# timsu1104/Open-vocabulary-3D-Object-Detection

Measured on AMD Instinct MI355X. Metric: scenes/sec (train step) SUN RGB-D 20k pts nqueries=128, higher is better.
Workload: dtype bf16; 1 GPU; SUN RGB-D train step, bs=8/GPU, 20000 pts, nqueries=128, 3DETR 256-d enc3/dec8, text-emb 640, AdamW + clip 0.1; global_batch=8, points=20000, parallelism=dp1

## Files before the change

include/ov3d.h:

```cpp
#ifndef OV3D_H_
#define OV3D_H_

#include <stdint.h>

#ifdef __cplusplus
extern "C" {
#endif

#define OV3D_OK 0
#define OV3D_EINVAL (-1)
#define OV3D_ELAUNCH (-2)

const char* ov3d_version(void);

int ov3d_fps(const float* xyz, int B, int N, int M, int32_t* idx_out, float* new_xyz_out,
             float* workspace, void* stream);
long long ov3d_fps_workspace(int B, int N);
int ov3d_fps_pair_status(const float* workspace, int B, int N, int M, int32_t* status,
                         void* stream);

int ov3d_nbr_max_fwd(const void* y, long long P, int S, int C, void* out, uint8_t* arg,
                     void* stream);
int ov3d_nbr_max_bwd(const void* g, const uint8_t* arg, long long P, int S, int C, void* dy,
                     void* stream);
// ... 195 lines not shown
int ov3d_rows256_supported(long long M, int N, int K);
int ov3d_rows256(const void* X, long long ldx, int K, int N, const void* W, long long ldw, void* Y,
                 long long ldy, long long M, unsigned int* counters, void* stream);
int ov3d_rows256_bn(const void* X, long long ldx, const float* scale, const float* shift,
                    const void* W, long long ldw, void* Y, long long ldy, void* Z, long long ldz,
                    long long M, unsigned int* counters, void* stream);

typedef struct {
    const void* W;
    long long ldw;
    const void* bias;
    void* out;
    long long ldo;
    int N;
    int sel;
} ov3d_lngemm_problem;
int ov3d_lngemm_supported(int R, int C, int N);
int ov3d_lngemm_fwd(int R, const void* src, int src_bf16, const void* y, float dropout_p,
                    const int64_t* seed, int site, const float* ga, const float* ba,
                    const void* pos, int pos_bf16, const float* gb, const float* bb, float eps,
                    float* s, float* mean, float* rstd, void* xa, void* xap, void* xb, int xb_bf16,
                    long long xb_inner, long long xb_s0, long long xb_s1, int nprob,
                    const ov3d_lngemm_problem* probs, int epilogue, float dropout_p2,
                    const int64_t* seed2, int site2, void* stream);
int ov3d_lngemm_bwd_parts(int R);
int ov3d_lngemm_stamps_arm(void* buf);
int ov3d_lngemm_bwd(int R, const float* s, const float* mean, const float* rstd, const float* ds,
                    const void* dxa, const void* dxap, const void* dxb, int dxb_bf16,
                    long long dxb_inner, long long dxb_s0, long long dxb_s1, const float* ga,
                    const float* gb, float dropout_p, const int64_t* seed, int site, float* dsrc,
                    void* dy, void* dpos, int dpos_bf16, float* partials, int accumulate,
                    const void* W, long long ldw, int N, int epilogue, float dropout_p2,
                    const void* H, long long ldh, void* dx, long long lddx, void* stream);

int ov3d_attn_fwd(const void* q, const void* k, const void* v, long long sq, long long sk,
                  long long sv, int B, int H, int Lq, int Lk, float scale, float dropout_p,
                  const int64_t* seed, int site, void* o, long long so, float* lse,
                  uint32_t* dropbits, float* workspace, int nsplit, void* stream);
long long ov3d_attn_fwd_workspace(int B, int H, int Lq, int Lk, int nsplit);
long long ov3d_attn_dropbits_words(int B, int H, int Lq, int Lk);
int ov3d_attn_bwd(const void* q, const void* k, const void* v, long long sq, long long sk,
                  long long sv, const void* o, long long so, const void* dout, long long sdo,
                  const float* lse, int B, int H, int Lq, int Lk, float scale, float dropout_p,
                  const uint32_t* dropbits, float* dvec, void* dq, long long sdq, void* dk,
                  long long sdk, void* dv, long long sdv, float* workspace, int nsplit,
                  void* stream);

typedef struct {
    const void* q; long long sq; const void* k; long long sk; const void* v; long long sv;
    const void* dout; long long sdo; const float* lse; const float* dvec;
    const uint32_t* dropbits; void* dk; long long sdk; void* dv; long long sdv;
} ov3d_attn_dkdv_job;
int ov3d_attn_bwd_dkdv_batch(const ov3d_attn_dkdv_job* jobs, int njobs, int B, int H, int Lq,
                             int Lk, float scale, float dropout_p, void* stream);

int ov3d_attn_small_bwd(int on);

long long ov3d_attn_maskbits_words(int B, int Lq, int Lk);
int ov3d_attn_mask_pack(const void* src, int kind, float thr, int B, int Lq, int Lk,
                        uint32_t* words, void* stream);
int ov3d_attn_fwd_masked(const void* q, const void* k, const void* v, long long sq, long long sk,
                         long long sv, int B, int H, int Lq, int Lk, float scale, float dropout_p,
                         const int64_t* seed, int site, void* o, long long so, float* lse,
                         uint32_t* dropbits, float* workspace, int nsplit,
                         const uint32_t* maskbits, void* stream);
int ov3d_attn_fwd_pregen(const void* q, const void* k, const void* v, long long sq, long long sk,
// ... 267 lines not shown
```

open-vocabulary-3d-object-detection_amd/_native.py:

```python
import ctypes
import os

import torch

_HERE = os.path.dirname(os.path.abspath(__file__))
LIB_PATH = os.path.join(_HERE, "lib", "libov3d_hip.so")

OV3D_GIOU_CYTHON = 0
OV3D_GIOU_TENSOR = 1

_lib = None

_SIGS = {
    "ov3d_fps": "piiipppp",
    "ov3d_fps_pair_status": "piiipp",
    "ov3d_ball_query": "ppiiifipp",
    "ov3d_ball_query_cells": "ppiiifipplp",
    "ov3d_group_fwd": "ppplllpiiiiifipp",
    "ov3d_group_bwd": "ppiiiiilllpp",
    "ov3d_gather_fwd": "ppiiiipp",
    "ov3d_gather_bwd": "ppiiiipp",
    "ov3d_giou3d": "pppiiiiipipp",
    "ov3d_giou3d_bwd_aligned": "pppiiippp",
    "ov3d_giou3d_bwd": "pppiiiipppp",
# ... 65 lines not shown
    "ov3d_resnorm_bwd": "lipppppppilllppfpippipipippppip",
    "ov3d_rows_gemm": "iiiplplipplp",
    "ov3d_bn_stats_finalize": "piidppffpppppppp",
    "ov3d_colsum_group": "pipiip",
    "ov3d_sa_dy_fused": "ppppiiiipppppppppppip",
    "ov3d_sa_dy2_fused": "pppppppppppppppiiipppip",
    "ov3d_bn_bwd_stats_finalize": "piidppppppppp",
    "ov3d_rows_gemm_act": "iiiplplipifpiplplp",
    "ov3d_rows_gemm_group": "iipip",
    "ov3d_tile_gemm": "iiiplplipplp",
    "ov3d_tile_gemm_act": "iiiplplipifpiplplp",
    "ov3d_tile_gemm2": "iiiplpliplpliplp",
    "ov3d_tile_gemm_batched": "iiiipllpllipllp",
    "ov3d_sun_aug_points": "pilippiipippp",
    "ov3d_sun_aug_boxes": "plpppiipipippp",
    "ov3d_sun_cuboid_eval": "piipppiiippippppp",
    "ov3d_sun_crop_sample": "piipppiippipppp",
    "ov3d_sun_labels": "pip",
    "ov3d_box_points_count": "pllipiipp",
    "ov3d_box3d_iou_eval": "ppppiiipp",
    "ov3d_ap_match": "ppppiiiidpp",
    "ov3d_ap_curve": "plppiplppp",
    "ov3d_project_box2d": "pppliipppppp",
    "ov3d_heads_out_fwd": "plippipiippippppppipp",
    "ov3d_heads_out_bwd": "pppiiiipiippppppplp",
    "ov3d_gemm256": "plplpiplpliiiip",
    "ov3d_conv3x3_gemm256": "piiiiplpiplpliip",
    "ov3d_gemm256_pair": "pplpplppippliiip",
    "ov3d_gemm256_batched": "pllpllpliplliiiiip",
    "ov3d_lngemm_fwd": "ipipfpipppippfppppppilllipifpip",
    "ov3d_rows256": "pliiplpllpp",
    "ov3d_rows256_bn": "plppplplpllpp",
    "ov3d_lngemm_bwd": "ipppppppilllppfpipppipipliifplplp",
}
EXPORTS = tuple(_SIGS) + ("ov3d_version", "ov3d_sa_layer_supported", "ov3d_attn_fwd_workspace",
                          "ov3d_attn_dropbits_words", "ov3d_attn_maskbits_words", "ov3d_fps_workspace", "ov3d_attn_small_bwd", "ov3d_set_loss_fwd_parts",
                          "ov3d_wgrad_workspace", "ov3d_wgrad_tiles", "ov3d_wgrad_group_tiles",
                          "ov3d_set_loss_desc_size",
                          "ov3d_resnorm_supported", "ov3d_resnorm_bwd_parts",
                          "ov3d_adamw_chunk", "ov3d_wgrad_group_workspace",
                          "ov3d_rows_gemm_supported", "ov3d_sa_dy_fused_supported",
                          "ov3d_tile_gemm_supported", "ov3d_sun_range_parts", "ov3d_heads_out_max_text",
                          "ov3d_heads_out_workspace", "ov3d_stamps_arm", "ov3d_stamps_count",
                          "ov3d_stamps_get", "ov3d_wall_clock_khz",
                          "ov3d_attnpool_fused_supported", "ov3d_lngemm_supported",
                          "ov3d_lngemm_bwd_parts", "ov3d_lngemm_stamps_arm", "ov3d_stream_create",
                          "ov3d_ball_query_ws_bytes", "ov3d_rows256_supported")

_CT = {"p": ctypes.c_void_p, "i": ctypes.c_int, "l": ctypes.c_longlong, "f": ctypes.c_float,
       "d": ctypes.c_double}


class NativeError(RuntimeError):
    pass


def load():
    global _lib
    if _lib is None:
        if not os.path.exists(LIB_PATH):
            raise NativeError(
                f"{LIB_PATH} not found: the HIP extension is required (no CPU fallback); "
                "build it with `make -C open-vocabulary-3d-object-detection_amd/csrc`")
        lib = ctypes.CDLL(LIB_PATH)
        for name, sig in _SIGS.items():
            fn = getattr(lib, name)
            fn.argtypes = [_CT[c] for c in sig]
            fn.restype = ctypes.c_int
        lib.ov3d_sa_layer_supported.argtypes = [ctypes.c_int, ctypes.c_int]
        lib.ov3d_sa_layer_supported.restype = ctypes.c_int
        lib.ov3d_attn_fwd_workspace.argtypes = [ctypes.c_int] * 5
        lib.ov3d_attn_fwd_workspace.restype = ctypes.c_longlong
        lib.ov3d_attn_dropbits_words.argtypes = [ctypes.c_int] * 4
        lib.ov3d_attn_dropbits_words.restype = ctypes.c_longlong
        lib.ov3d_set_loss_fwd_parts.argtypes = [ctypes.c_int] * 3
        lib.ov3d_set_loss_fwd_parts.restype = ctypes.c_longlong
        lib.ov3d_fps_workspace.argtypes = [ctypes.c_int] * 2
        lib.ov3d_fps_workspace.restype = ctypes.c_longlong
        lib.ov3d_stamps_arm.argtypes = [ctypes.c_void_p, ctypes.c_longlong, ctypes.c_longlong]
        lib.ov3d_stamps_arm.restype = ctypes.c_int
# ... 13 lines not shown
        lib.ov3d_wgrad_tiles.restype = ctypes.c_int
        lib.ov3d_wgrad_group_tiles.argtypes = [ctypes.c_int] * 2
        lib.ov3d_wgrad_group_tiles.restype = ctypes.c_int
        lib.ov3d_set_loss_desc_size.argtypes = []
        lib.ov3d_set_loss_desc_size.restype = ctypes.c_longlong
        lib.ov3d_resnorm_supported.argtypes = [ctypes.c_int]
        lib.ov3d_resnorm_supported.restype = ctypes.c_int
        lib.ov3d_resnorm_bwd_parts.argtypes = [ctypes.c_longlong, ctypes.c_int]
        lib.ov3d_resnorm_bwd_parts.restype = ctypes.c_int
        lib.ov3d_adamw_chunk.argtypes = []
        lib.ov3d_adamw_chunk.restype = ctypes.c_int
        lib.ov3d_wgrad_group_workspace.argtypes = [ctypes.c_void_p, ctypes.c_int]
        lib.ov3d_wgrad_group_workspace.restype = ctypes.c_longlong
        lib.ov3d_sa_dy_fused_supported.argtypes = [ctypes.c_int] * 2
        lib.ov3d_sa_dy_fused_supported.restype = ctypes.c_int
        lib.ov3d_rows_gemm_supported.argtypes = [ctypes.c_int] * 3
        lib.ov3d_rows256_supported.argtypes = [ctypes.c_longlong, ctypes.c_int, ctypes.c_int]
        lib.ov3d_rows256_supported.restype = ctypes.c_int
        lib.ov3d_rows_gemm_supported.restype = ctypes.c_int
        lib.ov3d_tile_gemm_supported.argtypes = [ctypes.c_int] * 3
        lib.ov3d_tile_gemm_supported.restype = ctypes.c_int
        lib.ov3d_sun_range_parts.argtypes = [ctypes.c_int]
        lib.ov3d_sun_range_parts.restype = ctypes.c_int
        lib.ov3d_heads_out_max_text.argtypes = []
        lib.ov3d_heads_out_max_text.restype = ctypes.c_int
        lib.ov3d_attnpool_fused_supported.argtypes = [ctypes.c_int] * 3
        lib.ov3d_attnpool_fused_supported.restype = ctypes.c_int
        lib.ov3d_lngemm_supported.argtypes = [ctypes.c_int] * 3
        lib.ov3d_lngemm_supported.restype = ctypes.c_int
        lib.ov3d_lngemm_bwd_parts.argtypes = [ctypes.c_int]
        lib.ov3d_lngemm_bwd_parts.restype = ctypes.c_int
        lib.ov3d_lngemm_stamps_arm.argtypes = [ctypes.c_void_p]
        lib.ov3d_lngemm_stamps_arm.restype = ctypes.c_int
        lib.ov3d_heads_out_workspace.argtypes = [ctypes.c_int] * 2
        lib.ov3d_heads_out_workspace.restype = ctypes.c_longlong
        lib.ov3d_stream_create.argtypes = [ctypes.c_void_p]
        lib.ov3d_ball_query_ws_bytes.argtypes = [ctypes.c_int] * 2
        lib.ov3d_ball_query_ws_bytes.restype = ctypes.c_longlong
        lib.ov3d_stream_create.restype = ctypes.c_int
        lib.ov3d_version.argtypes = []
        lib.ov3d_version.restype = ctypes.c_char_p
        _lib = lib
    return _lib


def version():
    return load().ov3d_version().decode()


def stream_create(device):
    with torch.cuda.device(device):
        h = ctypes.c_void_p()
        rc = load().ov3d_stream_create(ctypes.byref(h))
        if rc != 0 or not h.value:
            raise NativeError(f"ov3d_stream_create failed with status {rc}")
        return torch.cuda.ExternalStream(h.value, device=device)


def _stream(t):
    return ctypes.c_void_p(torch.cuda.current_stream(t.device).cuda_stream)


def _ptr(t):
    return ctypes.c_void_p(t.data_ptr()) if t is not None else ctypes.c_void_p(0)


# ... 139 lines not shown
```

open-vocabulary-3d-object-detection_amd/resnorm.py:

```python
import os
from collections import namedtuple

import torch
from torch import nn

from . import _native
from . import attention as flash
from . import gemm

Pending = namedtuple("Pending", "src y p site")
LinY = namedtuple("LinY", "x w b relu_p", defaults=(None,))


class FanIn:

    def __init__(self):
        self.n = 0
        self.seen = 0
        self.bufs = None

    def take(self):
        k = self.seen
        self.seen += 1
        last = self.seen == self.n
# ... 524 lines not shown
        bf = torch.bfloat16
        C = x.shape[-1]
        xc = x.reshape(-1, C)
        w1c, b1c = gemm.cast_param(w1, bf), gemm.cast_param(b1, bf)
        w2c, b2c = gemm.cast_param(w2, bf), gemm.cast_param(b2, bf)
        M, F, N = xc.shape[0], w1c.shape[0], w2c.shape[0]
        seed = flash._seed(x.device) if p > 0 else None
        h = gemm.act_gemm(xc, w1c, _bias(b1c), True, 1, p, seed, site)
        y = gemm.act_gemm(h, w2c, _bias(b2c), True)
        ctx.save_for_backward(xc, h, w1c, w2c)
        ctx.params = (w1, b1, w2, b2)
        ctx.meta = (float(p), x.shape, x.dtype)
        return y.view(*x.shape[:-1], N)

    @staticmethod
    def backward(ctx, dy):
        xc, h, w1c, w2c = ctx.saved_tensors
        w1, b1, w2, b2 = ctx.params
        p, xshape, xdt = ctx.meta
        need = ctx.needs_input_grad
        M, F, N = h.shape[0], h.shape[1], w2c.shape[0]
        dy = dy.reshape(-1, N).to(torch.bfloat16).contiguous()
        dy1 = gemm.act_gemm(dy, w2c, None, False, 2, p, h=h)
        dw2, db2 = gemm.linear_weight_grads(dy, h, w2, b2, need[3], need[4])
        dw1, db1 = gemm.linear_weight_grads(dy1, xc, w1, b1, need[1], need[2])
        dx = gemm.act_gemm(dy1, w1c, None, False).to(xdt).view(xshape) if need[0] else None
        return dx, dw1, db1, dw2, db2, None, None


def _bias(b):
    return b.contiguous() if b is not None else None


def _ffn_ok(x, linear1, linear2, activation):
    if not isinstance(activation, nn.ReLU):
        return False
    return ffn_weights_ok(x, linear1.weight, linear2.weight)


def ffn_weights_ok(x, w1, w2):
    if not (fused_ffn and x.is_cuda and x.dtype == torch.bfloat16
            and torch.is_autocast_enabled("cuda")
            and torch.get_autocast_dtype("cuda") == torch.bfloat16 and x.stride(-1) == 1
            and w1.dim() == 2 and w2.dim() == 2):
        return False
    xr = x.reshape(-1, x.shape[-1])
    bf = torch.bfloat16
    w1c, w2c = gemm.cast_param(w1, bf), gemm.cast_param(w2, bf)
    if not (gemm.act_gemm_ok(xr, w1c, True) and w2c.stride(1) == 1 and w2c.stride(0) % 8 == 0
            and w2c.data_ptr() % 16 == 0 and w2c.shape[1] == w1c.shape[0]):
        return False
    M, C, F, N = xr.shape[0], xr.shape[1], w1c.shape[0], w2c.shape[0]
    return gemm.shape_ok(M, N, F) and gemm.shape_ok(M, F, N) and gemm.shape_ok(M, C, F)


def ffn(x, linear1, linear2, activation, dropout, site):
    if _ffn_ok(x, linear1, linear2, activation):
        p = dropout.p if dropout.training else 0.0
        with torch.autocast("cuda", enabled=False):
            return _FFN.apply(x, linear1.weight, linear1.bias, linear2.weight, linear2.bias, p, site)
    h = ffn_act(gemm.rows_linear(x, linear1.weight, linear1.bias), activation, dropout, site)
    return gemm.rows_linear(h, linear2.weight, linear2.bias)


def ffn_weights(x, w1, b1, w2, b2):
    with torch.autocast("cuda", enabled=False):
# ... 14 lines not shown
```

open-vocabulary-3d-object-detection_amd/transformer.py:

```python
import os
from typing import Optional

import torch
import torch.nn.functional as F
from torch import Tensor, nn

from . import _native
from . import attention as flash
from . import resnorm as rn
from . import gemm
from .gemm import cast_param, in_projection, rows_linear
from .helpers import ACTIVATION_DICT, NORM_DICT, get_clones


class MultiheadAttention(nn.Module):

    def __init__(self, embed_dim, num_heads, dropout=0.0):
        super().__init__()
        if embed_dim % num_heads:
            raise ValueError("embed_dim must be divisible by num_heads")
        self.embed_dim, self.num_heads, self.dropout = embed_dim, num_heads, dropout
        self.head_dim = embed_dim // num_heads
        self.in_proj_weight = nn.Parameter(torch.empty(3 * embed_dim, embed_dim))
        self.in_proj_bias = nn.Parameter(torch.zeros(3 * embed_dim))
# ... 181 lines not shown
        if use_ffn:
            self.linear1 = nn.Linear(d_model, dim_feedforward, bias=ffn_use_bias)
            self.dropout = nn.Dropout(dropout)
            self.linear2 = nn.Linear(dim_feedforward, d_model, bias=ffn_use_bias)
            self.norm2 = NORM_DICT[norm_name](d_model)
            self.dropout2 = nn.Dropout(dropout)
        self.norm1 = NORM_DICT[norm_name](d_model)
        self.dropout1 = nn.Dropout(dropout)
        self.activation = ACTIVATION_DICT[activation]()
        self.normalize_before = normalize_before
        self.nhead = nhead

    def forward(self, src, src_mask: Optional[Tensor] = None, src_key_padding_mask=None,
                pos: Optional[Tensor] = None, return_attn_weights=False):
        if src_key_padding_mask is not None or return_attn_weights:
            raise NotImplementedError
        x = self.norm1(src)
        qk = x if pos is None else x + pos
        src = src + self.dropout1(self.self_attn(qk, qk, x, attn_mask=src_mask))
        if self.use_ffn:
            x = self.norm2(src)
            h = self.dropout(self.activation(rows_linear(x, self.linear1.weight, self.linear1.bias)))
            src = src + self.dropout2(rows_linear(h, self.linear2.weight, self.linear2.bias))
        return src

    def forward_fused(self, pend, src_mask=None, pos=None):
        p1, p2 = (self.dropout1.p, self.dropout2.p) if self.training else (0.0, 0.0)
        site1, site2, site_ffn = rn.sites(self, 3)
        s, x, xp, _ = rn.resnorm(pend, self.norm1, pos=pos, want_a=True, want_ap=pos is not None)
        qk = xp if pos is not None else x
        y = self.self_attn(qk, qk, x, attn_mask=src_mask, defer_out=self.use_ffn)
        if not self.use_ffn:
            return rn.Pending(s, y, p1, site1)
        s, x, _, _ = rn.resnorm(rn.Pending(s, y, p1, site1), self.norm2)
        y = rn.ffn(x, self.linear1, self.linear2, self.activation, self.dropout, site_ffn)
        return rn.Pending(s, y, p2, site2)

    def fused_ok(self, x):
        return rn.supported(x, self.norm1, self.norm2 if self.use_ffn else None)


class TransformerDecoderLayer(nn.Module):
    def __init__(self, d_model, nhead=4, dim_feedforward=256, dropout=0.1, dropout_attn=None,
                 activation="relu", normalize_before=True, norm_fn_name="ln"):
        super().__init__()
        if not normalize_before:
            raise NotImplementedError("the reference builds pre-norm layers only")
        self.self_attn = MultiheadAttention(d_model, nhead, dropout=dropout)
        self.multihead_attn = MultiheadAttention(d_model, nhead, dropout=dropout)
        self.norm1 = NORM_DICT[norm_fn_name](d_model)
        self.norm2 = NORM_DICT[norm_fn_name](d_model)
        self.norm3 = NORM_DICT[norm_fn_name](d_model)
        self.dropout1 = nn.Dropout(dropout)
        self.dropout2 = nn.Dropout(dropout)
        self.dropout3 = nn.Dropout(dropout)
        self.linear1 = nn.Linear(d_model, dim_feedforward)
        self.dropout = nn.Dropout(dropout)
        self.linear2 = nn.Linear(dim_feedforward, d_model)
        self.activation = ACTIVATION_DICT[activation]()
        self.normalize_before = normalize_before

    def forward(self, tgt, memory, tgt_mask=None, memory_mask=None, tgt_key_padding_mask=None,
                memory_key_padding_mask=None, pos=None, query_pos=None, return_attn_weights=False,
                memory_pos=None):
        if tgt_key_padding_mask is not None or memory_key_padding_mask is not None:
            raise NotImplementedError
# ... 295 lines not shown
```

Before: 1720 scenes/s.

## Fuse encoder attention out-proj, residual+LayerNorm and FFN into one kernel

```diff
diff --git a/include/ov3d.h b/include/ov3d.h
--- a/include/ov3d.h
+++ b/include/ov3d.h
@@ -251,6 +251,20 @@
                     void* dy, void* dpos, int dpos_bf16, float* partials, int accumulate,
                     const void* W, long long ldw, int N, int epilogue, float dropout_p2,
                     const void* H, long long ldh, void* dx, long long lddx, void* stream);
+
+int ov3d_enc_post_supported(int R, int C, int F);
+int ov3d_enc_post_fwd(int R, const float* s, const void* o, const void* Wo, long long ldwo,
+                      const void* bo, float p1, const int64_t* seed, int site1, const float* g2,
+                      const float* be2, float eps, const void* W1, long long ldw1, const void* b1,
+                      float pf, int site_ffn, const void* W2, long long ldw2, const void* b2,
+                      int k_quarters, float* s1, float* mean, float* rstd, void* x2, void* h,
+                      void* y2, void* stream);
+int ov3d_enc_post_bwd(int R, const float* ds1, const void* dy2, const float* s1, const float* mean,
+                      const float* rstd, const void* h, const float* g2, const void* Wo,
+                      long long ldwo, const void* W1, long long ldw1, const void* W2,
+                      long long ldw2, float p1, const int64_t* seed, int site1, float pf,
+                      int k_quarters, float* ds, void* dy1, void* dout, void* d1, float* partials,
+                      int nparts, void* stream);
 
 int ov3d_attn_fwd(const void* q, const void* k, const void* v, long long sq, long long sk,
                   long long sv, int B, int H, int Lq, int Lk, float scale, float dropout_p,
diff --git a/open-vocabulary-3d-object-detection_amd/_native.py b/open-vocabulary-3d-object-detection_amd/_native.py
--- a/open-vocabulary-3d-object-detection_amd/_native.py
+++ b/open-vocabulary-3d-object-detection_amd/_native.py
@@ -121,6 +121,8 @@
     "ov3d_rows256": "pliiplpllpp",
     "ov3d_rows256_bn": "plppplplpllpp",
     "ov3d_lngemm_bwd": "ipppppppilllppfpipppipipliifplplp",
+    "ov3d_enc_post_fwd": "ippplpfpippfplpfiplpippppppp",
+    "ov3d_enc_post_bwd": "ipppppppplplplfpifipppppip",
 }
 EXPORTS = tuple(_SIGS) + ("ov3d_version", "ov3d_sa_layer_supported", "ov3d_attn_fwd_workspace",
                           "ov3d_attn_dropbits_words", "ov3d_attn_maskbits_words", "ov3d_fps_workspace", "ov3d_attn_small_bwd", "ov3d_set_loss_fwd_parts",
@@ -134,7 +136,8 @@
                           "ov3d_stamps_get", "ov3d_wall_clock_khz",
                           "ov3d_attnpool_fused_supported", "ov3d_lngemm_supported",
                           "ov3d_lngemm_bwd_parts", "ov3d_lngemm_stamps_arm", "ov3d_stream_create",
-                          "ov3d_ball_query_ws_bytes", "ov3d_rows256_supported")
+                          "ov3d_ball_query_ws_bytes", "ov3d_rows256_supported",
+                          "ov3d_enc_post_supported")
 
 _CT = {"p": ctypes.c_void_p, "i": ctypes.c_int, "l": ctypes.c_longlong, "f": ctypes.c_float,
        "d": ctypes.c_double}
@@ -214,6 +217,8 @@
         lib.ov3d_lngemm_bwd_parts.restype = ctypes.c_int
         lib.ov3d_lngemm_stamps_arm.argtypes = [ctypes.c_void_p]
         lib.ov3d_lngemm_stamps_arm.restype = ctypes.c_int
+        lib.ov3d_enc_post_supported.argtypes = [ctypes.c_int] * 3
+        lib.ov3d_enc_post_supported.restype = ctypes.c_int
         lib.ov3d_heads_out_workspace.argtypes = [ctypes.c_int] * 2
         lib.ov3d_heads_out_workspace.restype = ctypes.c_longlong
         lib.ov3d_stream_create.argtypes = [ctypes.c_void_p]
diff --git a/open-vocabulary-3d-object-detection_amd/csrc/encpost.hip b/open-vocabulary-3d-object-detection_amd/csrc/encpost.hip
--- /dev/null
+++ b/open-vocabulary-3d-object-detection_amd/csrc/encpost.hip
@@ -0,0 +1,748 @@
+#include "common.h"
+#include "rowdrop.h"
+#include "rowsum.h"
+
+#include <type_traits>
+
+namespace {
+
+typedef __bf16 bf16;
+typedef __bf16 bf16x8 __attribute__((ext_vector_type(8)));
+typedef __bf16 bf16x4 __attribute__((ext_vector_type(4)));
+typedef float f32x16 __attribute__((ext_vector_type(16)));
+typedef short s16x4 __attribute__((ext_vector_type(4)));
+
+constexpr int C = 256;
+constexpr int F = 128;
+constexpr int FWD_BM = 64, BWD_BM = 32;
+constexpr int RMULT = 64;
+constexpr int BK = 64;
+constexpr int LDI = C + 8, LDH = F + 8, LDW = BK + 8;
+constexpr int LDIB = C + 4, LDHB = F + 4, LDWB = C + 32, LDWBF = F + 32;
+constexpr int WSZ = C * LDW;
+static_assert(BK * LDWB <= WSZ && 16 * 2 * C * 2 <= WSZ && RMULT % FWD_BM == 0 && RMULT % BWD_BM == 0,
+              "W chunk region");
+
+__device__ __forceinline__ f32x16 mfma(bf16x8 a, bf16x8 b, f32x16 c) {
+    return __builtin_amdgcn_mfma_f32_32x32x16_bf16(a, b, c, 0, 0, 0);
+}
+__device__ __forceinline__ bf16x4 tr16(const bf16* p) {
+    s16x4 r = __builtin_amdgcn_ds_read_tr16_b64_v4i16((__attribute__((address_space(3))) s16x4*)(p));
+    return __builtin_bit_cast(bf16x4, r);
+}
+
+template <int NTL, int K, bool QS>
+struct Chain {
+    f32x16 acc[NTL], s01[NTL], s23[NTL];
+    __device__ __forceinline__ void zero() {
+#pragma unroll
+        for (int nt = 0; nt < NTL; ++nt)
+#pragma unroll
+            for (int v = 0; v < 16; ++v) acc[nt][v] = 0.f;
+    }
+    __device__ __forceinline__ void close(int sg) {
+        if (!QS) return;
+        constexpr int SPQ = K / 64;
+        if ((sg + 1) % SPQ) return;
+        const int q = (sg + 1) / SPQ - 1;
+#pragma unroll
+        for (int nt = 0; nt < NTL; ++nt)
+#pragma unroll
+            for (int v = 0; v < 16; ++v) {
+                if (q == 0) {
+                    s01[nt][v] = acc[nt][v];
+                    acc[nt][v] = 0.f;
+                } else if (q == 1) {
+                    s01[nt][v] = s01[nt][v] + acc[nt][v];
+                    acc[nt][v] = 0.f;
+                } else if (q == 2) {
+                    s23[nt][v] = acc[nt][v];
+                    acc[nt][v] = 0.f;
+                } else {
+                    acc[nt][v] = s01[nt][v] + (s23[nt][v] + acc[nt][v]);
+                }
+            }
+    }
+};
+
+template <int NTL, int K, bool QS>
+__device__ __forceinline__ void mma_fwd(Chain<NTL, K, QS>& ch, const bf16* ap, const bf16* wp, int chunk) {
+#pragma unroll
+    for (int s = 0; s < BK / 16; ++s) {
+        const bf16x8 af = *reinterpret_cast<const bf16x8*>(ap + 16 * s);
+        bf16x8 wf[NTL];
+#pragma unroll
+        for (int nt = 0; nt < NTL; ++nt) wf[nt] = *reinterpret_cast<const bf16x8*>(wp + 32 * nt * LDW + 16 * s);
+#pragma unroll
+        for (int nt = 0; nt < NTL; ++nt) ch.acc[nt] = mfma(wf[nt], af, ch.acc[nt]);
+        ch.close(chunk * (BK / 16) + s);
+    }
+}
+
+template <int NTL, int K, bool QS, int LW>
+__device__ __forceinline__ void mma_bwd(Chain<NTL, K, QS>& ch, const bf16* ap, const bf16* wp, int chunk) {
+#pragma unroll
+    for (int s = 0; s < BK / 16; ++s) {
+        const bf16x4 lo = *reinterpret_cast<const bf16x4*>(ap + 16 * s);
+        const bf16x4 hi = *reinterpret_cast<const bf16x4*>(ap + 16 * s + 8);
+        const bf16x8 af = bf16x8{lo[0], lo[1], lo[2], lo[3], hi[0], hi[1], hi[2], hi[3]};
+        bf16x8 wf[NTL];
+#pragma unroll
+        for (int nt = 0; nt < NTL; ++nt) {
+            const bf16x4 wl = tr16(wp + 16 * s * LW + 32 * nt);
+            const bf16x4 wh = tr16(wp + (16 * s + 8) * LW + 32 * nt);
+            wf[nt] = bf16x8{wl[0], wl[1], wl[2], wl[3], wh[0], wh[1], wh[2], wh[3]};
+        }
+#pragma unroll
+        for (int nt = 0; nt < NTL; ++nt) ch.acc[nt] = mfma(wf[nt], af, ch.acc[nt]);
+        ch.close(chunk * (BK / 16) + s);
+    }
+}
+
+__device__ __forceinline__ void ld8f(const float* p, float* v) {
+    const float4 a = *reinterpret_cast<const float4*>(p);
+    const float4 b = *reinterpret_cast<const float4*>(p + 4);
+    v[0] = a.x; v[1] = a.y; v[2] = a.z; v[3] = a.w;
+    v[4] = b.x; v[5] = b.y; v[6] = b.z; v[7] = b.w;
+}
+__device__ __forceinline__ void st8f(float* p, const float* v) {
+    *reinterpret_cast<float4*>(p) = make_float4(v[0], v[1], v[2], v[3]);
+    *reinterpret_cast<float4*>(p + 4) = make_float4(v[4], v[5], v[6], v[7]);
+}
+
+struct FwdArgs {
+    const float* s; const bf16* o;
+    const bf16* Wo; long long ldwo; const bf16* bo;
+    uint32_t thresh1; float ks1; const int64_t* seed; uint32_t site1;
+    const float* g2; const float* be2; float eps;
+    const bf16* W1; long long ldw1; const bf16* b1;
+    uint32_t threshf; float ksf; uint32_t sitef;
+    const bf16* W2; long long ldw2; const bf16* b2;
+    float* s1; float* mean; float* rstd; bf16* x2; bf16* h; bf16* y2;
+};
+
+template <bool QS, int BM>
+__global__ __launch_bounds__(BM * 8, QS ? BM / 32 : BM / 16) void enc_post_fwd_kernel(FwdArgs a) {
+    constexpr int NT = BM * 8;
+    constexpr int RPP = NT / 32;
+    __shared__ __attribute__((aligned(16))) bf16 img[BM * LDI];
+    __shared__ __attribute__((aligned(16))) bf16 ws[WSZ];
+    __shared__ __attribute__((aligned(16))) bf16 bias_s[2 * C + F];
+    __shared__ __attribute__((aligned(16))) float ln_s[2 * C];
+    const int tid = threadIdx.x, wave = tid >> 6, lane = tid & 63, r32 = lane & 31, h = lane >> 5;
+    const int wm = wave >> 2, wn = wave & 3;
+    const int m0 = blockIdx.x * BM;
+    const int arow = wm * 32 + r32;
+
+    {
+        const int t = tid < 80 ? tid : 0;
+        const bf16* bsrc = t < 32 ? a.bo + 8 * t : t < 64 ? a.b2 + 8 * (t - 32) : a.b1 + 8 * (t - 64);
+        const bf16x8 bv = *reinterpret_cast<const bf16x8*>(bsrc);
+        const int u = tid & 127;
+        const float4 lv = *reinterpret_cast<const float4*>((u < 64 ? a.g2 : a.be2 - C) + 4 * u);
+        if (tid < 80) *reinterpret_cast<bf16x8*>(bias_s + 8 * tid) = bv;
+        if (tid < 128) *reinterpret_cast<float4*>(ln_s + 4 * tid) = lv;
+    }
+    const bf16* const bo_s = bias_s;
+    const bf16* const b2_s = bias_s + C;
+    const bf16* const b1_s = bias_s + 2 * C;
+
+    constexpr int NPC = C * BK / 8 / NT, NPF = F * BK / 8 / NT;
+    bf16x8 rw[NPC];
+    auto wload = [&](const bf16* W, long long ldw, int kc, int np) __attribute__((always_inline)) {
+#pragma unroll
+        for (int j = 0; j < NPC; ++j)
+            if (j < np) {
+                const int idx = tid + NT * j;
+                rw[j] = *reinterpret_cast<const bf16x8*>(W + (size_t)(idx >> 3) * ldw + kc + 8 * (idx & 7));
+            }
+    };
+    auto wstore = [&](int np) __attribute__((always_inline)) {
+#pragma unroll
+        for (int j = 0; j < NPC; ++j)
+            if (j < np) {
+                const int idx = tid + NT * j;
+                *reinterpret_cast<bf16x8*>(&ws[(idx >> 3) * LDW + 8 * (idx & 7)]) = rw[j];
+            }
+    };
+
+    {
+        bf16x8 ra[BM * C / 8 / NT];
+#pragma unroll
+        for (int j = 0; j < BM * C / 8 / NT; ++j) {
+            const int idx = tid + NT * j;
+            ra[j] = *reinterpret_cast<const bf16x8*>(a.o + (size_t)(m0 + (idx >> 5)) * C + 8 * (idx & 31));
+        }
+        wload(a.Wo, a.ldwo, 0, NPC);
+#pragma unroll
+        for (int j = 0; j < BM * C / 8 / NT; ++j) {
+            const int idx = tid + NT * j;
+            *reinterpret_cast<bf16x8*>(&img[(idx >> 5) * LDI + 8 * (idx & 31)]) = ra[j];
+        }
+        wstore(NPC);
+    }
+    __syncthreads();
+
+    const uint32_t smix1 = a.thresh1 ? rowdrop::seed_mix(a.seed, a.site1) : 0u;
+    const bool dropf = a.threshf != 0;
+    const uint32_t smixf = dropf ? rowdrop::seed_mix(a.seed, a.sitef) : 0u;
+
+    {
+        Chain<2, C, QS> ch;
+        ch.zero();
+        const bf16* ap = img + arow * LDI + 8 * h;
+        const bf16* wp = ws + (wn * 64 + r32) * LDW + 8 * h;
+#pragma unroll
+        for (int c = 0; c < C / BK; ++c) {
+            if (c + 1 < C / BK) wload(a.Wo, a.ldwo, BK * (c + 1), NPC);
+            else wload(a.W1, a.ldw1, 0, NPF);
+            mma_fwd(ch, ap + BK * c, wp, c);
+            __syncthreads();
+            if (c + 1 < C / BK) {
+                wstore(NPC);
+                __syncthreads();
+            }
+        }
+#pragma unroll
+        for (int nt = 0; nt < 2; ++nt)
+#pragma unroll
+            for (int g = 0; g < 4; ++g) {
+                const int col = wn * 64 + 32 * nt + 8 * g + 4 * h;
+                const bf16x4 bb = *reinterpret_cast<const bf16x4*>(bo_s + col);
+                bf16x4 o;
+#pragma unroll
+                for (int q = 0; q < 4; ++q) o[q] = (bf16)(ch.acc[nt][4 * g + q] + (float)bb[q]);
+                *reinterpret_cast<bf16x4*>(&img[arow * LDI + col]) = o;
+            }
+        wstore(NPF);
+    }
+    __syncthreads();
+
+    wload(a.W1, a.ldw1, BK, NPF);
+    {
+        const int c = (tid & 31) * 8, lr0 = tid >> 5;
+        float sv[4][8];
+#pragma unroll
+        for (int it = 0; it < 4; ++it) ld8f(a.s + (size_t)(m0 + lr0 + RPP * it) * C + c, sv[it]);
+        float ga[8], ba[8];
+        ld8f(ln_s + c, ga);
+        ld8f(ln_s + C + c, ba);
+#pragma unroll
+        for (int it = 0; it < 4; ++it) {
+            const int lr = lr0 + RPP * it;
+            const long long r = m0 + lr;
+            const size_t off = (size_t)r * C + c;
+            float* s = sv[it];
+            const bf16x8 yv = *reinterpret_cast<const bf16x8*>(&img[lr * LDI + c]);
+            float y[8];
+#pragma unroll
+            for (int j = 0; j < 8; ++j) y[j] = (float)yv[j];
+            if (a.thresh1) {
+                bool keep[8];
+                rowdrop::keep8(rowdrop::row_base(smix1, r), c, a.thresh1, keep);
+#pragma unroll
+                for (int j = 0; j < 8; ++j) {
+                    const float d = (float)(bf16)(y[j] * a.ks1);
+                    s[j] += keep[j] ? d : 0.f;
+                }
+            } else {
+#pragma unroll
+                for (int j = 0; j < 8; ++j) s[j] += y[j];
+            }
+            st8f(a.s1 + off, s);
+            float t = 0.f;
+#pragma unroll
+            for (int j = 0; j < 8; ++j) t += s[j];
+            const float mu = row_sum32_lanes(t) / (float)C;
+            float q = 0.f;
+#pragma unroll
+            for (int j = 0; j < 8; ++j) q += (s[j] - mu) * (s[j] - mu);
+            const float rs = rsqrtf(row_sum32_lanes(q) / (float)C + a.eps);
+            if (c == 0) {
+                a.mean[r] = mu;
+                a.rstd[r] = rs;
+            }
+            bf16x8 xo;
+#pragma unroll
+            for (int j = 0; j < 8; ++j) {
+                const float xh = (s[j] - mu) * rs;
+                xo[j] = (bf16)(xh * ga[j] + ba[j]);
+            }
+            *reinterpret_cast<bf16x8*>(a.x2 + off) = xo;
+            *reinterpret_cast<bf16x8*>(&img[lr * LDI + c]) = xo;
+        }
+    }
+    __syncthreads();
+
+    {
+        Chain<1, C, QS> ch;
+        ch.zero();
+        const bf16* ap = img + arow * LDI + 8 * h;
+        const bf16* wp = ws + (wn * 32 + r32) * LDW + 8 * h;
+#pragma unroll
+        for (int c = 0; c < C / BK; ++c) {
+            if (c > 0) {
+                if (c + 1 < C / BK) wload(a.W1, a.ldw1, BK * (c + 1), NPF);
+                else wload(a.W2, a.ldw2, 0, NPC);
+            }
+            mma_fwd(ch, ap + BK * c, wp, c);
+            __syncthreads();
+            if (c + 1 < C / BK) {
+                wstore(NPF);
+                __syncthreads();
+            }
+        }
+        const uint32_t rbase = dropf ? rowdrop::row_base(smixf, m0 + arow) : 0u;
+#pragma unroll
+        for (int g = 0; g < 4; ++g) {
+            const int col = wn * 32 + 8 * g + 4 * h;
+            const bf16x4 bb = *reinterpret_cast<const bf16x4*>(b1_s + col);
+            bf16x4 o;
+#pragma unroll
+            for (int q = 0; q < 4; ++q) o[q] = (bf16)(ch.acc[0][4 * g + q] + (float)bb[q]);
+            bool keep[4] = {true, true, true, true};
+            if (dropf) {
+#pragma unroll
+                for (int j = 0; j < 4; j += 2) {
+                    const uint32_t hs = rowdrop::mix24(rbase + (uint32_t)((col + j) >> 1) * 0x27D4EB2Fu);
+                    keep[j] = (hs & 0xffffu) >= a.threshf;
+                    keep[j + 1] = (hs >> 16) >= a.threshf;
+                }
+            }
+#pragma unroll
+            for (int q = 0; q < 4; ++q) {
+                const float rr = fmaxf((float)o[q], 0.f);
+                o[q] = keep[q] ? (bf16)(rr * a.ksf) : (bf16)0.f;
+            }
+            *reinterpret_cast<bf16x4*>(&img[arow * LDH + col]) = o;
+        }
+        wstore(NPC);
+    }
+    __syncthreads();
+    wload(a.W2, a.ldw2, BK, NPC);
+#pragma unroll
+    for (int j = 0; j < BM * F / 8 / NT; ++j) {
+        const int idx = tid + NT * j, r = idx >> 4, pc = idx & 15;
+        *reinterpret_cast<bf16x8*>(a.h + (size_t)(m0 + r) * F + 8 * pc) =
+            *reinterpret_cast<const bf16x8*>(&img[r * LDH + 8 * pc]);
+    }
+
+    {
+        Chain<2, F, QS> ch;
+        ch.zero();
+        const bf16* ap = img + arow * LDH + 8 * h;
+        const bf16* wp = ws + (wn * 64 + r32) * LDW + 8 * h;
+#pragma unroll
+        for (int c = 0; c < F / BK; ++c) {
+            mma_fwd(ch, ap + BK * c, wp, c);
+            __syncthreads();
+            if (c + 1 < F / BK) {
+                wstore(NPC);
+                __syncthreads();
+            }
+        }
+#pragma unroll
+        for (int nt = 0; nt < 2; ++nt)
+#pragma unroll
+            for (int g = 0; g < 4; ++g) {
+                const int col = wn * 64 + 32 * nt + 8 * g + 4 * h;
+                const bf16x4 bb = *reinterpret_cast<const bf16x4*>(b2_s + col);
+                bf16x4 o;
+#pragma unroll
+                for (int q = 0; q < 4; ++q) o[q] = (bf16)(ch.acc[nt][4 * g + q] + (float)bb[q]);
+                *reinterpret_cast<bf16x4*>(&img[arow * LDI + col]) = o;
+            }
+    }
+    __syncthreads();
+#pragma unroll
+    for (int j = 0; j < BM * C / 8 / NT; ++j) {
+        const int idx = tid + NT * j, r = idx >> 5, pc = idx & 31;
+        *reinterpret_cast<bf16x8*>(a.y2 + (size_t)(m0 + r) * C + 8 * pc) =
+            *reinterpret_cast<const bf16x8*>(&img[r * LDI + 8 * pc]);
+    }
+}
+
+struct BwdArgs {
+    const float* ds1; const bf16* dy2;
+    const float* s1; const float* mean; const float* rstd;
+    const bf16* h; const float* g2;
+    const bf16* Wo; long long ldwo;
+    const bf16* W1; long long ldw1;
+    const bf16* W2; long long ldw2;
+    uint32_t thresh1; float ks1; const int64_t* seed; uint32_t site1;
+    float ksf;
+    float* ds; bf16* dy1; bf16* dout; bf16* d1; float* partials;
+};
+
+template <bool QS, bool IT4, int BM>
+__global__ __launch_bounds__(BM * 8, QS ? BM / 32 : BM / 16) void enc_post_bwd_kernel(BwdArgs a) {
+    constexpr int NT = BM * 8;
+    constexpr int RPP = NT / 32;
+    __shared__ __attribute__((aligned(16))) bf16 img[BM * LDI];
+    __shared__ __attribute__((aligned(16))) bf16 ws[WSZ];
+    __shared__ __attribute__((aligned(16))) float g2_s[C];
+    float* const red = reinterpret_cast<float*>(ws);
+    const int tid = threadIdx.x, wave = tid >> 6, lane = tid & 63, r32 = lane & 31, h = lane >> 5;
+    const int wm = wave >> 2, wn = wave & 3;
+    const int m0 = blockIdx.x * BM;
+    const int arow = wm * 32 + r32;
+    const int gq = lane >> 4, i16 = lane & 15;
+    const int trow = 4 * (gq >> 1) + (i16 >> 2), tcol = 16 * (gq & 1) + 4 * (i16 & 3);
+
+    {
+        const float4 lv = *reinterpret_cast<const float4*>(a.g2 + 4 * (tid & 63));
+        if (tid < 64) *reinterpret_cast<float4*>(g2_s + 4 * tid) = lv;
+    }
+
+    bf16x8 rw[BK * C / 8 / NT];
+    auto wload = [&](const bf16* W, long long ldw, int kc, auto n_c) __attribute__((always_inline)) {
+        constexpr int N = decltype(n_c)::value;
+#pragma unroll
+        for (int j = 0; j < BK * N / 8 / NT; ++j) {
+            const int idx = tid + NT * j, k = idx / (N / 8), pc = idx % (N / 8);
+            rw[j] = *reinterpret_cast<const bf16x8*>(W + (size_t)(kc + k) * ldw + 8 * pc);
+        }
+    };
+    auto wstore = [&](auto n_c) __attribute__((always_inline)) {
+        constexpr int N = decltype(n_c)::value;
+#pragma unroll
+        for (int j = 0; j < BK * N / 8 / NT; ++j) {
+            const int idx = tid + NT * j, k = idx / (N / 8), pc = idx % (N / 8);
+            *reinterpret_cast<bf16x8*>(&ws[k * (N + 32) + 8 * pc]) = rw[j];
+        }
+    };
+    using NF = std::integral_constant<int, F>;
+    using NC = std::integral_constant<int, C>;
+
+    {
+        bf16x8 ra[BM * C / 8 / NT];
+#pragma unroll
+        for (int j = 0; j < BM * C / 8 / NT; ++j) {
+            const int idx = tid + NT * j;
+            ra[j] = *reinterpret_cast<const bf16x8*>(a.dy2 + (size_t)(m0 + (idx >> 5)) * C + 8 * (idx & 31));
+        }
+        wload(a.W2, a.ldw2, 0, NF{});
+#pragma unroll
+        for (int j = 0; j < BM * C / 8 / NT; ++j) {
+            const int idx = tid + NT * j;
+            bf16* d = &img[(idx >> 5) * LDIB + 8 * (idx & 31)];
+            const bf16x8 v = ra[j];
+            *reinterpret_cast<bf16x4*>(d) = bf16x4{v[0], v[1], v[2], v[3]};
+            *reinterpret_cast<bf16x4*>(d + 4) = bf16x4{v[4], v[5], v[6], v[7]};
+        }
+        wstore(NF{});
+    }
+    __syncthreads();
+
+    {
+        Chain<1, C, QS> ch;
+        ch.zero();
+        const bf16* ap = img + arow * LDIB + 4 * h;
+        const bf16* wp = ws + trow * LDWBF + wn * 32 + tcol;
+        bf16x4 hv[4];
+#pragma unroll
+        for (int c = 0; c < C / BK; ++c) {
+            if (c + 1 < C / BK) {
+                wload(a.W2, a.ldw2, BK * (c + 1), NF{});
+            } else {
+                wload(a.W1, a.ldw1, 0, NC{});
+#pragma unroll
+                for (int g = 0; g < 4; ++g)
+                    hv[g] = *reinterpret_cast<const bf16x4*>(a.h + (size_t)(m0 + arow) * F + wn * 32 + 8 * g + 4 * h);
+            }
+            mma_bwd<1, C, QS, LDWBF>(ch, ap + BK * c, wp, c);
+            __syncthreads();
+            if (c + 1 < C / BK) {
+                wstore(NF{});
+                __syncthreads();
+            }
+        }
+#pragma unroll
+        for (int g = 0; g < 4; ++g) {
+            const int col = wn * 32 + 8 * g + 4 * h;
+            bf16x4 o;
+#pragma unroll
+            for (int q = 0; q < 4; ++q) {
+                const bf16 v = (bf16)(ch.acc[0][4 * g + q] + 0.f);
+                o[q] = (float)hv[g][q] > 0.f ? (bf16)((float)v * a.ksf) : (bf16)0.f;
+            }
+            *reinterpret_cast<bf16x4*>(&img[arow * LDHB + col]) = o;
+        }
+        wstore(NC{});
+    }
+    __syncthreads();
+    wload(a.W1, a.ldw1, BK, NC{});
+#pragma unroll
+    for (int j = 0; j < BM * F / 8 / NT; ++j) {
+        const int idx = tid + NT * j, r = idx >> 4, pc = idx & 15;
+        const bf16* sp = &img[r * LDHB + 8 * pc];
+        const bf16x4 lo = *reinterpret_cast<const bf16x4*>(sp), hi = *reinterpret_cast<const bf16x4*>(sp + 4);
+        *reinterpret_cast<bf16x8*>(a.d1 + (size_t)(m0 + r) * F + 8 * pc) =
+            bf16x8{lo[0], lo[1], lo[2], lo[3], hi[0], hi[1], hi[2], hi[3]};
+    }
+
+    {
+        Chain<2, F, QS> ch;
+        ch.zero();
+        const bf16* ap = img + arow * LDHB + 4 * h;
+        const bf16* wp = ws + trow * LDWB + wn * 64 + tcol;
+#pragma unroll
+        for (int c = 0; c < F / BK; ++c) {
+            if (c + 1 == F / BK) wload(a.Wo, a.ldwo, 0, NC{});
+            mma_bwd<2, F, QS, LDWB>(ch, ap + BK * c, wp, c);
+            __syncthreads();
+            if (c + 1 < F / BK) {
+                wstore(NC{});
+                __syncthreads();
+            }
+        }
+#pragma unroll
+        for (int nt = 0; nt < 2; ++nt)
+#pragma unroll
+            for (int g = 0; g < 4; ++g) {
+                const int col = wn * 64 + 32 * nt + 8 * g + 4 * h;
+                bf16x4 o;
+#pragma unroll
+                for (int q = 0; q < 4; ++q) o[q] = (bf16)(ch.acc[nt][4 * g + q] + 0.f);
+                *reinterpret_cast<bf16x4*>(&img[arow * LDIB + col]) = o;
+            }
+    }
+    __syncthreads();
+
+    {
+        const int c = (tid & 31) * 8, ph = tid >> 5;
+        const uint32_t sm = a.thresh1 ? rowdrop::seed_mix(a.seed, a.site1) : 0u;
+        float ga[8];
+        ld8f(g2_s + c, ga);
+        float acc0[8], acc1[8];
+#pragma unroll
+        for (int j = 0; j < 8; ++j) acc0[j] = acc1[j] = 0.f;
+        float gv[4][8], svv[4][8], mu4[4], rs4[4];
+#pragma unroll
+        for (int it = 0; it < 4; ++it) {
+            if (!(it & 1)) {
+#pragma unroll
+                for (int u = it; u < it + 2; ++u) {
+                    const int lu = IT4 ? 32 * (ph >> 3) + (ph & 7) + 8 * u : ph + RPP * u;
+                    const size_t offu = (size_t)(m0 + lu) * C + c;
+                    ld8f(a.ds1 + offu, gv[u]);
+                    ld8f(a.s1 + offu, svv[u]);
+                    mu4[u] = a.mean[m0 + lu];
+                    rs4[u] = a.rstd[m0 + lu];
+                }
+            }
+            const int lr = IT4 ? 32 * (ph >> 3) + (ph & 7) + 8 * it : ph + RPP * it;
+            const long long r = m0 + lr;
+            const size_t off = (size_t)r * C + c;
+            float* g = gv[it];
+            const float* sv = svv[it];
+            const float mu = mu4[it], rs = rs4[it];
+            float da[8];
+            {
+                const bf16* sp = &img[lr * LDIB + c];
+                const bf16x4 lo = *reinterpret_cast<const bf16x4*>(sp), hi = *reinterpret_cast<const bf16x4*>(sp + 4);
+#pragma unroll
+                for (int j = 0; j < 4; ++j) {
+                    da[j] = (float)lo[j];
+                    da[4 + j] = (float)hi[j];
+                }
+            }
+            float xh[8], dxh[8], s1 = 0.f, s2 = 0.f;
+            float t0[8], t1[8];
+#pragma unroll
+            for (int j = 0; j < 8; ++j) {
+                xh[j] = (sv[j] - mu) * rs;
+                dxh[j] = da[j] * ga[j] + 0.f;
+                s1 += dxh[j];
+                s2 += dxh[j] * xh[j];
+                t0[j] = da[j] * xh[j];
+                t1[j] = da[j];
+            }
+            s1 = row_sum32_lanes(s1) / (float)C;
+            s2 = row_sum32_lanes(s2) / (float)C;
+#pragma unroll
+            for (int j = 0; j < 8; ++j) g[j] += rs * (dxh[j] - s1 - xh[j] * s2);
+            st8f(a.ds + off, g);
+            float d[8];
+            if (a.thresh1) {
+                bool keep[8];
+                rowdrop::keep8(rowdrop::row_base(sm, r), c, a.thresh1, keep);
+#pragma unroll
+                for (int j = 0; j < 8; ++j) d[j] = keep[j] ? g[j] * a.ks1 : 0.f;
+            } else {
+#pragma unroll
+                for (int j = 0; j < 8; ++j) d[j] = g[j];
+            }
+            bf16x8 dv;
+#pragma unroll
+            for (int j = 0; j < 8; ++j) dv[j] = (bf16)d[j];
+            *reinterpret_cast<bf16x8*>(a.dy1 + off) = dv;
+            {
+                bf16* dp = &img[lr * LDIB + c];
+                *reinterpret_cast<bf16x4*>(dp) = bf16x4{dv[0], dv[1], dv[2], dv[3]};
+                *reinterpret_cast<bf16x4*>(dp + 4) = bf16x4{dv[4], dv[5], dv[6], dv[7]};
+            }
+            if (IT4) {
+#pragma unroll
+                for (int j = 0; j < 8; ++j) {
+                    acc0[j] += t0[j];
+                    acc1[j] += t1[j];
+                }
+            } else {
+#pragma unroll
+                for (int j = 0; j < 8; ++j) {
+                    red[ph * C + c + j] = 0.f + t0[j];
+                    red[(RPP + ph) * C + c + j] = 0.f + t1[j];
+                }
+                __syncthreads();
+                {
+                    const int blk = tid >> 8, col = tid & 255;
+                    float u0 = 0.f, u1 = 0.f;
+#pragma unroll
+                    for (int p = 0; p < 8; ++p) {
+                        u0 += red[(8 * blk + p) * C + col];
+                        u1 += red[(RPP + 8 * blk + p) * C + col];
+                    }
+                    float* pp = a.partials + ((size_t)(m0 / 8) + (RPP / 8) * it + blk) * 4 * C;
+                    pp[col] = u0;
+                    pp[C + col] = u1;
+                    pp[2 * C + col] = 0.f;
+                    pp[3 * C + col] = 0.f;
+                }
+                __syncthreads();
+            }
+        }
+        if (IT4) {
+#pragma unroll
+            for (int j = 0; j < 8; ++j) {
+                red[ph * C + c + j] = acc0[j];
+                red[(RPP + ph) * C + c + j] = acc1[j];
+            }
+            __syncthreads();
+            {
+                const int blk = tid >> 8, col = tid & 255;
+                float u0 = 0.f, u1 = 0.f;
+#pragma unroll
+                for (int p = 0; p < 8; ++p) {
+                    u0 += red[(8 * blk + p) * C + col];
+                    u1 += red[(RPP + 8 * blk + p) * C + col];
+                }
+                float* pp = a.partials + ((size_t)(m0 / 32) + blk) * 4 * C;
+                pp[col] = u0;
+                pp[C + col] = u1;
+                pp[2 * C + col] = 0.f;
+                pp[3 * C + col] = 0.f;
+            }
+            __syncthreads();
+        }
+    }
+    wstore(NC{});
+    __syncthreads();
+
+    {
+        Chain<2, C, QS> ch;
+        ch.zero();
+        const bf16* ap = img + arow * LDIB + 4 * h;
+        const bf16* wp = ws + trow * LDWB + wn * 64 + tcol;
+#pragma unroll
+        for (int c = 0; c < C / BK; ++c) {
+            if (c + 1 < C / BK) wload(a.Wo, a.ldwo, BK * (c + 1), NC{});
+            mma_bwd<2, C, QS, LDWB>(ch, ap + BK * c, wp, c);
+            __syncthreads();
+            if (c + 1 < C / BK) {
+                wstore(NC{});
+                __syncthreads();
+            }
+        }
+#pragma unroll
+        for (int nt = 0; nt < 2; ++nt)
+#pragma unroll
+            for (int g = 0; g < 4; ++g) {
+                const int col = wn * 64 + 32 * nt + 8 * g + 4 * h;
+                bf16x4 o;
+#pragma unroll
+                for (int q = 0; q < 4; ++q) o[q] = (bf16)(ch.acc[nt][4 * g + q] + 0.f);
+                *reinterpret_cast<bf16x4*>(&img[arow * LDIB + col]) = o;
+            }
+    }
+    __syncthreads();
+#pragma unroll
+    for (int j = 0; j < BM * C / 8 / NT; ++j) {
+        const int idx = tid + NT * j, r = idx >> 5, pc = idx & 31;
+        const bf16* sp = &img[r * LDIB + 8 * pc];
+        const bf16x4 lo = *reinterpret_cast<const bf16x4*>(sp), hi = *reinterpret_cast<const bf16x4*>(sp + 4);
+        *reinterpret_cast<bf16x8*>(a.dout + (size_t)(m0 + r) * C + 8 * pc) =
+            bf16x8{lo[0], lo[1], lo[2], lo[3], hi[0], hi[1], hi[2], hi[3]};
+    }
+}
+
+bool al16(const void* p) { return ((uintptr_t)p & 15) == 0; }
+bool bad_p(float p) { return !(p >= 0.f && p < 1.f); }
+bool bad_w(const void* W, long long ldw, int K) { return !W || !al16(W) || ldw % 8 || ldw < K; }
+
+}
+
+extern "C" int ov3d_enc_post_supported(int R, int C_, int F_) {
+    return R > 0 && R % RMULT == 0 && C_ == C && F_ == F;
+}
+
+extern "C" int ov3d_enc_post_fwd(int R, const float* s, const void* o, const void* Wo, long long ldwo,
+                                 const void* bo, float p1, const int64_t* seed, int site1,
+                                 const float* g2, const float* be2, float eps, const void* W1,
+                                 long long ldw1, const void* b1, float pf, int site_ffn,
+                                 const void* W2, long long ldw2, const void* b2, int k_quarters,
+                                 float* s1, float* mean, float* rstd, void* x2, void* h, void* y2,
+                                 void* stream) {
+    if (!ov3d_enc_post_supported(R, C, F) || !s || !o || !bo || !g2 || !be2 || !b1 || !b2 || !s1 ||
+        !mean || !rstd || !x2 || !h || !y2)
+        return OV3D_EINVAL;
+    if (bad_p(p1) || bad_p(pf) || ((p1 > 0.f || pf > 0.f) && !seed)) return OV3D_EINVAL;
+    if (bad_w(Wo, ldwo, C) || bad_w(W1, ldw1, C) || bad_w(W2, ldw2, F)) return OV3D_EINVAL;
+    if (!al16(s) || !al16(o) || !al16(bo) || !al16(g2) || !al16(be2) || !al16(b1) || !al16(b2) ||
+        !al16(s1) || !al16(x2) || !al16(h) || !al16(y2))
+        return OV3D_EINVAL;
+    FwdArgs a{s, (const bf16*)o, (const bf16*)Wo, ldwo, (const bf16*)bo, rowdrop::thresh(p1),
+              1.f / (1.f - p1), seed, (uint32_t)site1, g2, be2, eps, (const bf16*)W1, ldw1,
+              (const bf16*)b1, rowdrop::thresh(pf), 1.f / (1.f - pf), (uint32_t)site_ffn,
+              (const bf16*)W2, ldw2, (const bf16*)b2, s1, mean, rstd, (bf16*)x2, (bf16*)h, (bf16*)y2};
+    hipStream_t st = ov3d_stream(stream);
+    constexpr int BM = FWD_BM;
+    if (k_quarters) enc_post_fwd_kernel<true, BM><<<R / BM, BM * 8, 0, st>>>(a);
+    else enc_post_fwd_kernel<false, BM><<<R / BM, BM * 8, 0, st>>>(a);
+    OV3D_LAUNCH_CHECK();
+    return OV3D_OK;
+}
+
+extern "C" int ov3d_enc_post_bwd(int R, const float* ds1, const void* dy2, const float* s1,
+                                 const float* mean, const float* rstd, const void* h, const float* g2,
+                                 const void* Wo, long long ldwo, const void* W1, long long ldw1,
+                                 const void* W2, long long ldw2, float p1, const int64_t* seed,
+                                 int site1, float pf, int k_quarters, float* ds, void* dy1,
+                                 void* dout, void* d1, float* partials, int nparts, void* stream) {
+    if (!ov3d_enc_post_supported(R, C, F) || !ds1 || !dy2 || !s1 || !mean || !rstd || !h || !g2 ||
+        !ds || !dy1 || !dout || !d1 || !partials)
+        return OV3D_EINVAL;
+    if (bad_p(p1) || bad_p(pf) || (p1 > 0.f && !seed)) return OV3D_EINVAL;
+    if (bad_w(Wo, ldwo, C) || bad_w(W1, ldw1, C) || bad_w(W2, ldw2, F)) return OV3D_EINVAL;
+    if (!al16(ds1) || !al16(dy2) || !al16(s1) || !al16(h) || !al16(g2) || !al16(ds) || !al16(dy1) ||
+        !al16(dout) || !al16(d1) || !al16(partials))
+        return OV3D_EINVAL;
+    const bool it4 = R >= 4096;
+    if (nparts != ov3d_resnorm_bwd_parts(R, C) || nparts != R / (it4 ? 32 : 8)) return OV3D_EINVAL;
+    BwdArgs a{ds1, (const bf16*)dy2, s1, mean, rstd, (const bf16*)h, g2, (const bf16*)Wo, ldwo,
+              (const bf16*)W1, ldw1, (const bf16*)W2, ldw2, rowdrop::thresh(p1), 1.f / (1.f - p1),
+              seed, (uint32_t)site1, 1.f / (1.f - pf), ds, (bf16*)dy1, (bf16*)dout, (bf16*)d1,
+              partials};
+    hipStream_t st = ov3d_stream(stream);
+    constexpr int BM = BWD_BM, NT = BM * 8;
+    const int grid = R / BM;
+    if (k_quarters) {
+        if (it4) enc_post_bwd_kernel<true, true, BM><<<grid, NT, 0, st>>>(a);
+        else enc_post_bwd_kernel<true, false, BM><<<grid, NT, 0, st>>>(a);
+    } else {
+        if (it4) enc_post_bwd_kernel<false, true, BM><<<grid, NT, 0, st>>>(a);
+        else enc_post_bwd_kernel<false, false, BM><<<grid, NT, 0, st>>>(a);
+    }
+    OV3D_LAUNCH_CHECK();
+    return OV3D_OK;
+}
diff --git a/open-vocabulary-3d-object-detection_amd/resnorm.py b/open-vocabulary-3d-object-detection_amd/resnorm.py
--- a/open-vocabulary-3d-object-detection_amd/resnorm.py
+++ b/open-vocabulary-3d-object-detection_amd/resnorm.py
@@ -580,6 +580,134 @@
     return b.contiguous() if b is not None else None
 
 
+_ENC_POST = os.environ.get("OV3D_ENC_POST", "1")
+enc_post = _ENC_POST != "0"
+enc_post_fwd = _ENC_POST != "bwd"
+enc_post_bwd = _ENC_POST != "fwd"
+
+
+def _al16(t):
+    return t if (t.is_contiguous() and t.data_ptr() % 16 == 0) else t.contiguous().clone()
+
+
+class _EncPost(torch.autograd.Function):
+
+    @staticmethod
+    def forward(ctx, meta, s, o, wo, bo, g2, be2, w1, b1, w2, b2):
+        p1, pf, site1, site_ffn, eps, shape = meta
+        bf = torch.bfloat16
+        C = shape[-1]
+        sr = s.reshape(-1, C).contiguous()
+        orr = o.reshape(-1, C).contiguous()
+        R = sr.shape[0]
+        dev = sr.device
+        woc, w1c, w2c = gemm.cast_param(wo, bf), gemm.cast_param(w1, bf), gemm.cast_param(w2, bf)
+        boc, b1c, b2c = (_al16(gemm.cast_param(b, bf)) for b in (bo, b1, b2))
+        F = w1c.shape[0]
+        kq = int(gemm.ROWS_GEMM and R <= gemm.ROWS_GEMM_MAX_M)
+        seed = flash._seed(dev) if (p1 > 0 or pf > 0) else None
+        s1 = torch.empty((R, C), dtype=torch.float32, device=dev)
+        mean = torch.empty(R, dtype=torch.float32, device=dev)
+        rstd = torch.empty(R, dtype=torch.float32, device=dev)
+        x2 = torch.empty((R, C), dtype=bf, device=dev)
+        if enc_post_fwd:
+            h = torch.empty((R, F), dtype=bf, device=dev)
+            y2 = torch.empty((R, C), dtype=bf, device=dev)
+            _native.call("ov3d_enc_post_fwd", R, sr, orr, woc, woc.stride(0), boc, float(p1), seed,
+                         site1, g2, be2, float(eps), w1c, w1c.stride(0), b1c, float(pf), site_ffn,
+                         w2c, w2c.stride(0), b2c, kq, s1, mean, rstd, x2, h, y2, like=sr)
+        else:
+            y1 = gemm.act_gemm(orr, woc, boc, True)
+            _native.call("ov3d_resnorm_fwd", R, C, sr, 0, y1, 1, float(p1), seed if p1 > 0 else None,
+                         site1, g2, be2, None, 0, None, None, float(eps), s1, mean, rstd, x2, None,
+                         None, 0, 0, 0, 0, like=sr)
+            h = gemm.act_gemm(x2, w1c, b1c, True, 1, pf, seed if pf > 0 else None, site_ffn)
+            y2 = gemm.act_gemm(h, w2c, b2c, True)
+        ctx.save_for_backward(s1, mean, rstd, g2, None, orr, x2, h, woc, w1c, w2c)
+        ctx.seed = seed if p1 > 0 else None
+        ctx.params = (g2, be2, None, None)
+        ctx.lin = (wo, bo, w1, b1, w2, b2)
+        ctx.meta = (p1, site1, R, C, shape, torch.float32, bf, None)
+        ctx.fans = (None, None)
+        ctx.ffn = (float(pf), kq, s.dtype, o.dtype)
+        return s1.view(shape), y2.view(shape)
+
+    @staticmethod
+    def backward(ctx, ds1, dy2):
+        s1, mean, rstd, g2, _, orr, x2, h, woc, w1c, w2c = ctx.saved_tensors
+        wo, bo, w1, b1, w2, b2 = ctx.lin
+        be2 = ctx.params[1]
+        p1, site1, R, C, shape = ctx.meta[:5]
+        pf, kq, sdt, odt = ctx.ffn
+        need = ctx.needs_input_grad
+        bf = torch.bfloat16
+        dev = s1.device
+        dy2r = dy2.reshape(R, C).to(bf).contiguous()
+        if not enc_post_bwd:
+            d1 = gemm.act_gemm(dy2r, w2c, None, False, 2, pf, h=h)
+            dw2, db2 = gemm.linear_weight_grads(dy2r, h, w2, b2, need[9], need[10])
+            dw1, db1 = gemm.linear_weight_grads(d1, x2, w1, b1, need[7], need[8])
+            dx2 = gemm.act_gemm(d1, w1c, None, False)
+            ds, dy1, _, dg2, dbe2, _, _ = _bwd_core(
+                ctx, ds1, dx2, None, None, (False, True, True, False, need[5], need[6], False, False))
+            ds, dy1 = ds.reshape(R, C), dy1.reshape(R, C)
+            dout = gemm._dgrad(dy1, woc)
+        else:
+            lib = _native.load()
+            nparts = lib.ov3d_resnorm_bwd_parts(R, C)
+            ds1r = ds1.reshape(R, C).to(torch.float32).contiguous()
+            ds = torch.empty((R, C), dtype=torch.float32, device=dev)
+            dy1 = torch.empty((R, C), dtype=bf, device=dev)
+            dout = torch.empty((R, C), dtype=bf, device=dev)
+            d1 = torch.empty((R, h.shape[1]), dtype=bf, device=dev)
+            partials = torch.empty((nparts, 4, C), dtype=torch.float32, device=dev)
+            _native.call("ov3d_enc_post_bwd", R, ds1r, dy2r, s1, mean, rstd, h, g2, woc,
+                         woc.stride(0), w1c, w1c.stride(0), w2c, w2c.stride(0), float(p1), ctx.seed,
+                         site1, float(pf), kq, ds, dy1, dout, d1, partials, nparts, like=s1)
+            dw2, db2 = gemm.linear_weight_grads(dy2r, h, w2, b2, need[9], need[10])
+            dw1, db1 = gemm.linear_weight_grads(d1, x2, w1, b1, need[7], need[8])
+            dg2 = dbe2 = None
+            slots = [(k, t) for k, t in ((0, g2), (1, be2)) if need[5 + k]]
+            if slots and gemm.DEFER_WGRAD and not torch.is_grad_enabled() and \
+                    gemm._leaf_param(g2) is g2 and gemm._leaf_param(be2) is be2:
+                gemm.defer_norm_grads(partials, nparts, C, slots)
+            elif slots:
+                dg2 = torch.empty(C, dtype=torch.float32, device=dev) if need[5] else None
+                dbe2 = torch.empty(C, dtype=torch.float32, device=dev) if need[6] else None
+                _colsums(partials, nparts, C, (dg2, dbe2, None, None), 0)
+        dwo, dbo = gemm.linear_weight_grads(dy1, orr, wo, bo, need[3], need[4])
+        ds = ds.view(shape).to(sdt) if need[1] else None
+        dout = dout.view(shape).to(odt) if need[2] else None
+        return None, ds, dout, dwo, dbo, dg2, dbe2, dw1, db1, dw2, db2
+
+
+def encoder_post(s, o, wo, bo, norm2, linear1, linear2, p1, pf, sites_):
+    if not (enc_post and enabled and fused_ffn and s is not None and s.is_cuda
+            and s.dtype == torch.float32 and o.dtype == torch.bfloat16 and o.shape == s.shape
+            and torch.is_autocast_enabled("cuda")
+            and torch.get_autocast_dtype("cuda") == torch.bfloat16):
+        return None
+    if bo is None or linear1.bias is None or linear2.bias is None or norm2 is None or \
+            not supported(s, norm2):
+        return None
+    shape = tuple(s.shape)
+    C = shape[-1]
+    R = s.numel() // C
+    F = linear1.weight.shape[0]
+    if tuple(wo.shape) != (C, C) or tuple(linear1.weight.shape) != (F, C) or \
+            tuple(linear2.weight.shape) != (C, F):
+        return None
+    if not _native.load().ov3d_enc_post_supported(R, C, F):
+        return None
+    if not (gemm.ROWS_GEMM and R <= gemm.ROWS_GEMM_MAX_M) and \
+            not (gemm.TILE_GEMM and gemm.ROWS_GEMM_MAX_M < R < gemm.GEMM256_MIN_M):
+        return None
+    meta = (float(p1), float(pf), int(sites_[0]), int(sites_[1]), norm2.eps, shape)
+    with torch.autocast("cuda", enabled=False):
+        return _EncPost.apply(meta, s, o, wo, bo, norm2.weight, norm2.bias, linear1.weight,
+                              linear1.bias, linear2.weight, linear2.bias)
+
+
 def _ffn_ok(x, linear1, linear2, activation):
     if not isinstance(activation, nn.ReLU):
         return False
diff --git a/open-vocabulary-3d-object-detection_amd/transformer.py b/open-vocabulary-3d-object-detection_amd/transformer.py
--- a/open-vocabulary-3d-object-detection_amd/transformer.py
+++ b/open-vocabulary-3d-object-detection_amd/transformer.py
@@ -237,6 +237,12 @@
         y = self.self_attn(qk, qk, x, attn_mask=src_mask, defer_out=self.use_ffn)
         if not self.use_ffn:
             return rn.Pending(s, y, p1, site1)
+        if isinstance(y, rn.LinY) and isinstance(self.activation, nn.ReLU):
+            pf = self.dropout.p if self.dropout.training else 0.0
+            r = rn.encoder_post(s, y.x, y.w, y.b, self.norm2, self.linear1, self.linear2, p1, pf,
+                                (site1, site_ffn))
+            if r is not None:
+                return rn.Pending(r[0], r[1], p2, site2)
         s, x, _, _ = rn.resnorm(rn.Pending(s, y, p1, site1), self.norm2)
         y = rn.ffn(x, self.linear1, self.linear2, self.activation, self.dropout, site_ffn)
         return rn.Pending(s, y, p2, site2)
```

Result: faster. 1764 scenes/s, median of 6 (+2.6%).
